# BerkIGuler/AdaFortiTran

Measured on AMD Instinct MI355X. Metric: OFDM frames/sec (120x14 grid, batch 128) + channel-estimation MSE vs reference, higher is better.
Workload: dtype f32; 1 GPU; C3: AdaFortiTran default config (6 layers, d=128, 4 heads, adaptive tokens), 120x14 grid, pilots 12x2; 128 frames per GPU per step; step = model(pilots_cpu, meta_cpu) through the module surface + device MSE partial; value = SURVEY 8(d)'s metric: H2D of pilots + meta INSIDE the step, output left on the device (= value_h2d_inclusive); the bare engine call on inputs resident in HBM is value_resident;; frames_per_gpu=128, global_batch=128, parallelism=frames sharded over 1 rank(s), lanes=1

## Files before the change

adafortitran_amd/csrc/attn16_device.h:

```cpp
#pragma once
#include <math.h>

#include <type_traits>

#include "attn_device.h"

namespace aft {

__device__ __forceinline__ f32x4 mfma16x4(float a, float b, f32x4 c) { return __builtin_amdgcn_mfma_f32_16x16x4f32(a, b, c, 0, 0, 0); }
__device__ __forceinline__ float srd_load1(Srd r, unsigned byte_off) {
    return __builtin_bit_cast(float, __builtin_amdgcn_raw_buffer_load_b32(r, byte_off, 0, 0));
}
__device__ __forceinline__ float groups_max(float x) {
    x = fmaxf(x, __shfl_xor(x, 16));
    return fmaxf(x, other_half(x));
}
__device__ __forceinline__ float groups_sum(float x) {
    x += __shfl_xor(x, 16);
    return x + other_half(x);
}

template <int TOK = 0, int HD = 16>
__device__ __forceinline__ void attn16_body(const float *__restrict__ q, const float *__restrict__ k, const float *__restrict__ vt,
                                            const float *__restrict__ qbias, float *__restrict__ out, int nblk, int tokens_rt,
                                            int tokpad_rt, int model_dim, float scale_log2e, const int first_task, const int total_waves,
                                            int ntasks, const int tail_task = -1) {
    int lane_l = threadIdx.x & 63;
    asm volatile("" : "+v"(lane_l));
    const int lane = lane_l, i = lane & 15, g = lane >> 4;
    const Srd qs = make_srd(q), ks = make_srd(k), vs = make_srd(vt), os = make_srd(out);
    const int tokens = TOK > 0 ? TOK : tokens_rt;
    const int tokpad = TOK > 0 ? (TOK + kTile - 1) / kTile * kTile : tokpad_rt;
    const int nkt = tokpad / kTile;
    const bool ragged = (tokens & (kTile - 1)) != 0;
    const unsigned blk_bytes = (unsigned)tokpad * kHeadDim * 4;
    static_assert(HD == 16 || HD == 8, "heads of 16 or 8 features");
    constexpr int NSUB = 32 / HD;
    auto first_block = [&](int task) { return (task / nkt) / NSUB; };
    auto sub_of = [&](int task) { return (task / nkt) & (NSUB - 1); };
    auto slot_of = [&](int sub) { return HD == 16 ? 2 * sub + (g >> 1) : sub; };
    const int vfeat = HD == 16 ? i : (i & 7);
    auto load_kq = [&](Srd src, int tile, f32x4 (&dst)[2], unsigned base, int sub) {
#pragma unroll
        for (int half = 0; half < 2; ++half)
            dst[half] = srd_load(src, base + (unsigned)(tile * 1024 + slot_of(sub) * 256 + (32 * (g & 1) + 16 * half + i) * 4) * 4u);
    };
    auto load_v = [&](int kt, f32x4 (&dst)[2], unsigned base, int sub) {
#pragma unroll
        for (int kb = 0; kb < 2; ++kb)
            dst[kb] = srd_load(vs, base + (unsigned)(kt * 1024 + (2 * kb + (g >> 1)) * 256 + (32 * (g & 1) + HD * sub + vfeat) * 4) * 4u);
    };
    auto mask_logits = [&](f32x4 (&sv)[2][2], int kt) {
#pragma unroll
        for (int kb = 0; kb < 2; ++kb)
#pragma unroll
            for (int v = 0; v < 4; ++v)
                if (kt * kTile + 16 * kb + 4 * g + v >= tokens) sv[kb][0][v] = sv[kb][1][v] = -INFINITY;
    };
    auto mask_values = [&](f32x4 (&vv)[2], int kt) {
#pragma unroll
        for (int kb = 0; kb < 2; ++kb)
#pragma unroll
            for (int v = 0; v < 4; ++v)
                if (kt * kTile + 16 * kb + 4 * g + v >= tokens) vv[kb][v] = 0.f;
    };
// ... 156 lines not shown
```

adafortitran_amd/csrc/attn_device.h:

```cpp
#pragma once
#include <math.h>

#include <type_traits>

#include "aft_internal.h"
#include "srd.h"

namespace aft {

#ifndef AFT_ATTN_WAVES
#define AFT_ATTN_WAVES 3
#endif

constexpr float kRescaleThreshold = 64.0f;
constexpr float kZeroRefThreshold = 32.0f;

__device__ __forceinline__ float other_half(float x) {
    const unsigned u = __builtin_bit_cast(unsigned, x);
    const auto r = __builtin_amdgcn_permlane32_swap(u, u, false, false);
    return __builtin_bit_cast(float, (threadIdx.x & 32) ? r[0] : r[1]);
}

__device__ __forceinline__ float max16(const f32x16 &v) {
    float m = __builtin_fmaxf(v[0], v[1]);
// ... 118 lines not shown
        }
#pragma unroll
        for (int e = 0; e < 16; ++e)
            if (kt * kTile + (e & 3) + 8 * (e >> 2) + 4 * h >= tokens) sv[e] = -INFINITY;
    };
    auto mask_values = [&](f32x4 (&vvb)[NB][4], int kt) {
      if (!BS && pad8) return;
#pragma unroll
      for (int b = 0; b < NB; ++b) {
        f32x4 (&vv)[4] = vvb[b];
        if constexpr (BS) {
#pragma unroll
            for (int sl = 0; sl < 4; ++sl) {
                bf16x8 e = __builtin_bit_cast(bf16x8, vv[sl]);
#pragma unroll
                for (int j = 0; j < 8; ++j)
                    if (kt * kTile + 16 * (sl >> 1) + 8 * (j >> 2) + 4 * h + (j & 3) >= tokens) e[j] = (__bf16)0.0f;
                vv[sl] = __builtin_bit_cast(f32x4, e);
            }
        } else {
#pragma unroll
            for (int g = 0; g < 4; ++g)
#pragma unroll
                for (int j = 0; j < 4; ++j)
                    if (kt * kTile + 8 * g + 4 * h + j >= tokens) vv[g][j] = 0.f;
        }
      }
    };

  const int rounds = SINK ? 1 : (ntasks + total_waves - 1) / total_waves + (tail_task >= 0 ? 1 : 0);
  int round = 0;
  int task = first_task < ntasks ? first_task : tail_task;
  f32x4 qreg[NQ][4], kcur[NQ][4], vcur[NB][4];
  if (task >= 0) {
      const unsigned hb0 = head_base(task);
      load_qk(qs, task % nkt, qreg, hb0, sub_of(task));
      load_qk(ks, 0, kcur, hb0, sub_of(task));
      load_tile(vs, 0, vcur, hb0, second_block_bytes(task));
  }
  for (; task >= 0; ++round) {
    ASTAMP(0);
#ifdef AFT_DIAG_STAMPS
    if (stamps && lane == 0) stamps[(size_t)task * 8 + 6] = __builtin_amdgcn_s_memrealtime();
#endif
    const int qt = task % nkt;
    const int pb = first_block(task);
    const int sub = sub_of(task);
    const unsigned hb = head_base(task);
    const unsigned vb1 = second_block_bytes(task);
    const int next_task = SINK || task >= ntasks ? -1 : (task + total_waves < ntasks ? task + total_waves : tail_task);
    const bool has_next = next_task >= 0;

    if constexpr (!BS) {
        const float *bq = qbias + (pb % nblk) * kHeadDim + 4 * h + (GEN ? 8 * sub : 0);
#pragma unroll
        for (int b = 0; b < NQ; ++b)
#pragma unroll
            for (int s = 0; s < 4; ++s)
                if (4 * b + s < (GEN ? NS : 4 * NB))
                    qreg[b][s] = (qreg[b][s] + *reinterpret_cast<const f32x4 *>(bq + 32 * b + 8 * s)) * scale_log2e;
    }
    if (ragged && qt == nkt - 1 && qt * kTile + r >= tokens) {
#pragma unroll
        for (int b = 0; b < NQ; ++b)
#pragma unroll
            for (int s = 0; s < 4; ++s)
                if (4 * b + s < (GEN ? NS : 4 * NB)) qreg[b][s] = f32x4{0.f, 0.f, 0.f, 0.f};
    }

    AttnRow<NB> st;
    f32x16 sA, sB;
    if constexpr (BS) sA = qk_tile_bs(kcur[0], qreg[0], true, 0.f, h);
    else sA = qk_tile<NQ, NMF>(kcur, qreg, true, a_one, 0.f);
    if (nkt > 1) load_qk(ks, 1, kcur, hb, sub);
    if (ragged && nkt == 1) { mask_logits(sA, 0); mask_values(vcur, 0); }
    {
        float m0 = max16(sA);
        m0 = fmaxf(m0, other_half(m0));
        if constexpr (BS) m0 = round_to_bf16(m0);
        st.zero_ref = !__any(fabsf(m0) > kZeroRefThreshold);
        st.m_ref = st.zero_ref ? 0.f : m0;
        if (!st.zero_ref) {
#pragma unroll
            for (int e = 0; e < 16; ++e) sA[e] -= m0;
        }
    }
#pragma unroll
    for (int b = 0; b < NB; ++b) st.oacc[b] = f32x16{0};
    st.lsum2 = f32x2{0.f, 0.f};
    ASTAMP(1);

    auto step = [&](auto fast, f32x16 &cur, f32x16 &nxt, int kt) {
        constexpr bool FAST = decltype(fast)::value;
        set_progress_priority((rounds - 1 - round) * nkt + (nkt - 1 - kt), rounds * nkt);
        const bool more = FAST || kt + 1 < nkt;
        if (more) {
            if constexpr (BS) nxt = qk_tile_bs(kcur[0], qreg[0], st.zero_ref, -st.m_ref, h);
            else nxt = qk_tile<NQ, NMF>(kcur, qreg, st.zero_ref, a_one, -st.m_ref);
            if (FAST || kt + 2 < nkt) load_qk(ks, kt + 2, kcur, hb, sub);
        } else if (has_next) {
            const unsigned hbn = head_base(next_task);
            load_qk(qs, next_task % nkt, qreg, hbn, sub_of(next_task));
            load_qk(ks, 0, kcur, hbn, sub_of(next_task));
        }
        const float tmax = max16(cur);
        if (__builtin_expect(__any(tmax > kRescaleThreshold), 0)) {
            const float tm = fmaxf(tmax, other_half(tmax));
            float grow = fmaxf(tm, 0.f);
            if constexpr (BS) grow = round_to_bf16(st.m_ref + grow) - st.m_ref;
            const float f = __builtin_amdgcn_exp2f(-grow);
            st.m_ref += grow;
            st.zero_ref = false;
#pragma unroll
// ... 94 lines not shown
```

adafortitran_amd/csrc/chain_device.h:

```cpp
#pragma once
#include "aft_internal.h"
#include "srd.h"

namespace aft {

template <int D>
struct ChainShape {
    static constexpr int WAVES = D / 32;
    static constexpr int THREADS = 64 * WAVES;
    static constexpr int XB = WAVES * 1024;
    static constexpr int HB = 2 * WAVES * 1024;
    static constexpr int ST = 32 * WAVES * 2;
    static constexpr int PAR = 4 * D;
    static constexpr size_t LDS_BYTES = sizeof(float) * (size_t)(XB + HB + ST + PAR);
};

struct ChainArgs {
    const float *attn;
    float *x;
    const float *wo, *w1, *w2, *wqkv;
    const float *bo, *b1, *b2, *g1, *be1, *g2, *be2;
    const float *bv;
    float *q, *k, *vt;
    int rows, tokens, tokpad, heads;
    int x_blocked;
    const float *lin2_w, *lin2_b;
    float *out6;
    int out6_features, out6_stride;
    const float *emb_conv, *emb_tok6, *emb_w1, *emb_b1, *emb_pos;
    int emb_S, emb_T, emb_p0, emb_p1, emb_K;
    unsigned long long *stamps;
    int tpp;
};

ChainArgs make_chain_args(const aft_config &c, const aft_layer_weights *mlp_w, const float *mlp_packed, const aft_layer_weights *qkv_w,
                          const float *qkv_packed, const float *attn, float *x, float *q, float *k, float *vt, int rows, int tokens,
                          int tokpad, const ChainFusion *fuse);

template <int NT, int PFS>
struct WRing {
    f32x4 b[PFS + 1][NT];
};


template <int NKB, int NT, int PFS, int TS>
__device__ __forceinline__ void ring_load(WRing<NT, PFS> &ring, Srd w, unsigned w_lane, int step) {
    const int kb = step >> 2, s = step & 3;
#pragma unroll
    for (int t = 0; t < NT; ++t)
        ring.b[step % (PFS + 1)][t] = srd_load_c(w, w_lane, (unsigned)((t * TS * NKB + kb) * 1024 + s * 256) * 4);
}

template <int NKB, int NT, int PFS, int TS>
__device__ __forceinline__ void gemm_preload(WRing<NT, PFS> &ring, Srd w, unsigned w_lane) {
#pragma unroll
    for (int p = 0; p < PFS && p < 4 * NKB; ++p) ring_load<NKB, NT, PFS, TS>(ring, w, w_lane, p);
    __builtin_amdgcn_sched_barrier(0);
}

template <int NKB, int NT, int PFS, int TS, unsigned NORMAL, class Act, unsigned ZERO = 0>
__device__ __forceinline__ void gemm_run(WRing<NT, PFS> &ring, Srd w, unsigned w_lane, f32x16 (&acc)[NT], Act act) {
#pragma unroll
    for (int step = 0; step < 4 * NKB; ++step) {
        if (step + PFS < 4 * NKB) ring_load<NKB, NT, PFS, TS>(ring, w, w_lane, step + PFS);
        __builtin_amdgcn_sched_barrier(0);
        const f32x4 a = act(step >> 2, step & 3);
#pragma unroll
        for (int t = 0; t < NT; ++t)
#pragma unroll
            for (int j = 0; j < 4; ++j) {
                const float wv = ring.b[step % (PFS + 1)][t][j];
                if (((ZERO >> t) & 1) && step == 0 && j == 0)
                    acc[t] = (NORMAL >> t) & 1 ? __builtin_amdgcn_mfma_f32_32x32x2f32(a[j], wv, f32x16{0}, 0, 0, 0)
                                               : __builtin_amdgcn_mfma_f32_32x32x2f32(wv, a[j], f32x16{0}, 0, 0, 0);
                else
                    acc[t] = (NORMAL >> t) & 1 ? __builtin_amdgcn_mfma_f32_32x32x2f32(a[j], wv, acc[t], 0, 0, 0)
                                               : __builtin_amdgcn_mfma_f32_32x32x2f32(wv, a[j], acc[t], 0, 0, 0);
            }
        __builtin_amdgcn_sched_barrier(0);
    }
}

__device__ __forceinline__ void bs_publish(float *buf, int block, int lane, const f32x16 &v) {
#pragma unroll
    for (int m = 0; m < 2; ++m) {
        const BsFrag f = bs_split(f32x4{v[8 * m], v[8 * m + 1], v[8 * m + 2], v[8 * m + 3]},
// ... 74 lines not shown

__device__ __forceinline__ f32x16 bias_acc(Srd bias, int f0, int h) {
    f32x16 acc;
#pragma unroll
    for (int s = 0; s < 4; ++s) {
        const f32x4 b = srd_load(bias, (unsigned)(f0 + 8 * s + 4 * h) * 4);
#pragma unroll
        for (int j = 0; j < 4; ++j) acc[4 * s + j] = b[j];
    }
    return acc;
}

#ifdef AFT_DIAG_STAMPS
#define STAMP(i)                                                                                               \
    do {                                                                                                       \
        if (a.stamps && tid == 0) a.stamps[(size_t)tile * 16 + (i)] = __builtin_amdgcn_s_memtime();    \
    } while (0)
#else
#define STAMP(i) do { } while (0)
#endif

struct ChainNoPre {
    __device__ __forceinline__ void operator()(int) const {}
};

template <int D, int ACT, bool MLP, bool QKV, bool BS = false, bool PT = false, class Pre = ChainNoPre>
__device__ __forceinline__ void chain_body(const ChainArgs &a, float *smem, const int tid_in, const int first_tile,
                                           const int tile_stride, const int tile_end, Pre pre = Pre{}) {
    using S = ChainShape<D>;
    constexpr int W = S::WAVES;
    static_assert(!PT || !BS, "plane-aligned tiles are instantiated for the fp32 body");
    int tid = tid_in;
    asm volatile("" : "+v"(tid));
    float *xb = smem;
    float *hb = xb + S::XB;
    float *stats = hb + S::HB;
    float *par = stats + S::ST;

    int lane = tid & 63;
    const int w = __builtin_amdgcn_readfirstlane(tid >> 6);
    int r = lane & 31, h = lane >> 5;
    const int fb = 32 * w;

    const Srd srd_wo = make_srd(a.wo), srd_w1 = make_srd(a.w1), srd_w2 = make_srd(a.w2), srd_wq = make_srd(a.wqkv);
    const Srd srd_attn = make_srd(a.attn), srd_x = make_srd(a.x);
    const Srd srd_bo = make_srd(a.bo), srd_b1 = make_srd(a.b1), srd_b2 = make_srd(a.b2);
    const Srd srd_q = make_srd(a.q), srd_k = make_srd(a.k), srd_vt = make_srd(a.vt);
    const unsigned wo_off = (unsigned)w * W * 1024 + lane * 4, w1_off = (unsigned)(2 * w) * W * 1024 + lane * 4;
    const unsigned w2_off = (unsigned)w * (2 * W) * 1024 + lane * 4;
    const unsigned wq_off = (unsigned)w * W * 1024 + lane * 4;
    const Srd srd_bv = make_srd(a.bv);

    if constexpr (MLP) {
        for (int i = tid; i < D; i += S::THREADS) {
            par[i] = a.g1[i];
            par[D + i] = a.be1[i];
            par[2 * D + i] = a.g2[i];
            par[3 * D + i] = a.be2[i];
        }
        __syncthreads();
    }
    constexpr int kEmbSteps = (kMaxPatchFeatures + 6 + 1) / 2;
    float *emb_w = hb + S::XB;
    int *emb_offs = reinterpret_cast<int *>(emb_w + D * (kMaxPatchFeatures + 6));
    if constexpr (!MLP) {
        if (a.emb_conv != nullptr) {
            const int pk = a.emb_p0 * a.emb_p1;
            for (int i = tid; i < D * a.emb_K; i += S::THREADS) emb_w[i] = a.emb_w1[i];
            for (int k = tid; k < a.emb_K; k += S::THREADS)
                emb_offs[k] = k < pk ? (k / a.emb_p1) * a.emb_T + k % a.emb_p1 : ~(k - pk);
            __syncthreads();
        }
    }
    const int ntiles = (a.rows + 31) / 32;
    const int rounds = (tile_end - first_tile + tile_stride - 1) / tile_stride;
    int round = 0;
#ifndef AFT_CHAIN_PFK
#define AFT_CHAIN_PFK 0
#endif
    constexpr int PFK = MLP ? (AFT_CHAIN_PFK < W ? AFT_CHAIN_PFK : W) : 0;
    constexpr bool AHEAD = AFT_CHAIN_PFK > 0;
    static_assert(!PT || !AHEAD, "plane-aligned tiles request a tile's operands at the tile's start");
    f32x4 of[MLP ? W : 1][4], xres[4];
    auto request_attn = [&](int t, int kb0, int kb1) {
        const unsigned ap = ((unsigned)t * W * 1024 + lane * 4) * 4;
#pragma unroll
        for (int kb = 0; kb < W; ++kb)
#pragma unroll
            for (int s = 0; s < 4; ++s)
                if (kb >= kb0 && kb < kb1) of[kb][s] = srd_load_c(srd_attn, ap, (unsigned)(kb * 1024 + s * 256) * 4);
    };
    auto request_x_pt = [&](int t, int valid) {
        const unsigned xr = ((unsigned)t * 32 * D + w * 1024 + (min(r, valid - 1) + 32 * h) * 4) * 4;
#pragma unroll
        for (int s = 0; s < 4; ++s) xres[s] = srd_load(srd_x, xr + 1024 * s);
    };
    auto request_x = [&](int t) {
        if (a.x_blocked) {
            const unsigned xr = ((unsigned)t * 32 * D + w * 1024 + lane * 4) * 4;
#pragma unroll
            for (int s = 0; s < 4; ++s) xres[s] = srd_load(srd_x, xr + 1024 * s);
        } else {
            const unsigned xr = ((unsigned)min(t * 32 + r, a.rows - 1) * D + fb + 4 * h) * 4;
#pragma unroll
            for (int s = 0; s < 4; ++s) xres[s] = srd_load(srd_x, xr + 32 * s);
        }
    };
    auto request_tile = [&](int t) {
        if constexpr (MLP) request_attn(t, 0, PFK);
        if (MLP || a.emb_conv == nullptr) request_x(t);
    };
    if (AHEAD && first_tile < ntiles) request_tile(first_tile);
    f32x16 emb_acc0;
    float emb_bv[kEmbSteps];
    auto emb_request = [&](int t) {
        int plane, tok;
        if constexpr (PT) {
            plane = t / a.tpp;
            tok = min((t - plane * a.tpp) * 32 + r, a.tokens - 1);
        } else {
            const int grow_n = min(t * 32 + r, a.rows - 1);
            plane = grow_n / a.tokens;
            tok = grow_n - plane * a.tokens;
        }
        const int tpr = a.emb_T / a.emb_p1, g = tok / tpr, tc = tok - g * tpr;
        const float *cplane = a.emb_conv + ((size_t)plane * a.emb_S + g * a.emb_p0) * a.emb_T + tc * a.emb_p1;
        const float *t6 = a.emb_tok6 ? a.emb_tok6 + ((size_t)(plane >> 1) * a.tokens + tok) * 6 : nullptr;
#pragma unroll
        for (int s = 0; s < 4; ++s) {
            const f32x4 b = *reinterpret_cast<const f32x4 *>(a.emb_b1 + fb + 8 * s + 4 * h);
            const f32x4 ps = *reinterpret_cast<const f32x4 *>(a.emb_pos + (size_t)tok * D + fb + 8 * s + 4 * h);
#pragma unroll
            for (int j = 0; j < 4; ++j) emb_acc0[4 * s + j] = b[j] + ps[j];
        }
#pragma unroll
        for (int st = 0; st < kEmbSteps; ++st) {
            const int k = 2 * st + h;
            emb_bv[st] = 0.f;
            if (k < a.emb_K) {
                const int off = emb_offs[k];
                emb_bv[st] = off >= 0 ? cplane[off] : t6[~off];
            }
        }
    };
    if constexpr (!MLP) {
        if (a.emb_conv != nullptr && first_tile < tile_end) emb_request(first_tile);
    }
    int pending_row0 = -1, pending_valid = 0;
    auto reduce_out6 = [&]() {
        const int P = a.out6_features;
        if (PT ? r < pending_valid : pending_row0 + r < a.rows) {
#pragma unroll
            for (int half = 0; half < 2; ++half) {
                const int f0 = 8 * half + 4 * h;
                if (f0 < P) {
                    f32x4 sum = *reinterpret_cast<const f32x4 *>(hb + lane * 8 + 4 * half);
#pragma unroll
                    for (int u = 1; u < W; ++u) {
                        const f32x4 t = *reinterpret_cast<const f32x4 *>(hb + (u * 64 + lane) * 8 + 4 * half);
                        sum += t;
                    }
#pragma unroll
                    for (int j = 0; j < 4; ++j) sum[j] += f0 + j < P ? a.lin2_b[f0 + j] : 0.f;
                    *reinterpret_cast<f32x4 *>(a.out6 + (size_t)(pending_row0 + r) * a.out6_stride + f0) = sum;
                }
            }
        }
    };
#pragma unroll 1
  for (int tile = first_tile; tile < tile_end; tile += tile_stride, ++round) {
    if constexpr (MLP && !QKV) {
        if (pending_row0 >= 0 && w == (round & (W - 1 < 3 ? W - 1 : 3))) reduce_out6();
    }
    pre(tile);
    if constexpr (PT && MLP) {
        int tid2 = tid_in;
        asm volatile("" : "+v"(tid2));
        lane = tid2 & 63;
        r = lane & 31;
        h = lane >> 5;
    }
#ifndef AFT_NO_PROGRESS_PRIORITY
    {
        const int left = rounds - 1 - round;
        if (left >= 3) __builtin_amdgcn_s_setprio(3);
        else if (left == 2) __builtin_amdgcn_s_setprio(2);
        else if (left == 1) __builtin_amdgcn_s_setprio(1);
        else __builtin_amdgcn_s_setprio(0);
    }
#endif
    const int row0 = tile * 32;
    const int grow = min(row0 + r, a.rows - 1);
    int plane_pt = 0, qt_pt = 0, valid_pt = 32;
    if constexpr (PT) {
        plane_pt = tile / a.tpp;
        qt_pt = tile - plane_pt * a.tpp;
        valid_pt = min(32, a.tokens - qt_pt * 32);
    }
    const bool row_ok = PT ? r < valid_pt : row0 + r < a.rows;
    const bool blocked = PT || a.x_blocked;
    const unsigned xrow = ((unsigned)grow * D + fb + 4 * h) * 4;
    unsigned lo = 0;
    asm volatile("" : "+v"(lo));
    const unsigned lo_lane = PT && MLP ? lo + lane * 4 : lo;
    const unsigned wo_lane = ((PT && MLP ? (unsigned)w * W * 1024 : wo_off) + lo_lane) * 4,
                   w1_lane = ((PT && MLP ? (unsigned)(2 * w) * W * 1024 : w1_off) + lo_lane) * 4,
                   w2_lane = ((PT && MLP ? (unsigned)w * (2 * W) * 1024 : w2_off) + lo_lane) * 4,
                   wq_lane = ((PT && MLP ? (unsigned)w * W * 1024 : wq_off) + lo_lane) * 4;
    STAMP(0);
#ifdef AFT_DIAG_STAMPS
    if (a.stamps && tid == 0) {
        a.stamps[(size_t)tile * 16 + 12] = __builtin_amdgcn_s_memrealtime();
        a.stamps[(size_t)tile * 16 + 14] = ((unsigned long long)__builtin_amdgcn_s_getreg((4 << 0) | (0 << 6) | (31 << 11)) << 32) |
                                           __builtin_amdgcn_s_getreg((20 << 0) | (0 << 6) | (31 << 11));
    }
#endif
#ifndef AFT_CHAIN_PFS
// ... 35 lines not shown
            bs_publish(xb, w, lane, cur);
        } else {
#pragma unroll
            for (int s = 0; s < 4; ++s)
                *reinterpret_cast<f32x4 *>(xb + (w * 4 + s) * 256 + lane * 4) = f32x4{cur[4 * s], cur[4 * s + 1], cur[4 * s + 2], cur[4 * s + 3]};
        }
        __syncthreads();
        STAMP(4);
        if constexpr (BS)
            gemm_run_bs<W, 2, PFF, 1, 0>(ring_ff, srd_w1, w1_lane, acc_h, [&](int kb, int m) { return bs_fetch(xb, kb, m, lane); });
        else
            gemm_run<W, 2, PFF, 1, 0>(ring_ff, srd_w1, w1_lane, acc_h, [&](int kb, int s) {
                return *reinterpret_cast<const f32x4 *>(xb + (kb * 4 + s) * 256 + lane * 4);
            });
        f32x16 acc_d[1] = {bias_acc(srd_b2, fb, h)};
        gemm_preload<2 * W, 1, PFD, 1>(ring_d, srd_w2, w2_lane);
        STAMP(5);
#pragma unroll
        for (int t = 0; t < 2; ++t) {
            f32x16 hid;
#pragma unroll
            for (int s = 0; s < 4; ++s) {
                const f32x2 g0 = activate2<ACT>(f32x2{acc_h[t][4 * s], acc_h[t][4 * s + 1]});
                const f32x2 g1 = activate2<ACT>(f32x2{acc_h[t][4 * s + 2], acc_h[t][4 * s + 3]});
                if constexpr (BS) {
                    hid[4 * s] = g0[0]; hid[4 * s + 1] = g0[1]; hid[4 * s + 2] = g1[0]; hid[4 * s + 3] = g1[1];
                } else {
                    *reinterpret_cast<f32x4 *>(hb + ((2 * w + t) * 4 + s) * 256 + lane * 4) = f32x4{g0[0], g0[1], g1[0], g1[1]};
                }
            }
            if constexpr (BS) bs_publish(hb, 2 * w + t, lane, hid);
        }
        __syncthreads();
        STAMP(6);
        if constexpr (BS)
            gemm_run_bs<2 * W, 1, PFD, 1, 0>(ring_d, srd_w2, w2_lane, acc_d, [&](int kb, int m) { return bs_fetch(hb, kb, m, lane); });
        else
            gemm_run<2 * W, 1, PFD, 1, 0>(ring_d, srd_w2, w2_lane, acc_d, [&](int kb, int s) {
                return *reinterpret_cast<const f32x4 *>(hb + (kb * 4 + s) * 256 + lane * 4);
            });
        if constexpr (QKV) gemm_preload<W, 3, PFQ, W>(ring_qkv, srd_wq, wq_lane);
#pragma unroll
        for (int e = 0; e < 16; ++e) cur[e] += acc_d[0][e];
        STAMP(7);
        layernorm_rows<D>(cur, stats, par + 2 * D + fb, par + 3 * D + fb, w, r, h);
        STAMP(8);
        if constexpr (!QKV) {
            if (AHEAD && tile + tile_stride < ntiles) request_tile(tile + tile_stride);
        }
        bool store_x = true;
        if constexpr (!QKV) {
            if (a.out6 != nullptr) {
                store_x = false;
                const int P = a.out6_features;
                f32x16 acc6 = f32x16{0};
#pragma unroll
                for (int s = 0; s < 4; ++s) {
                    f32x4 wv = {0.f, 0.f, 0.f, 0.f};
                    if (r < P) wv = *reinterpret_cast<const f32x4 *>(a.lin2_w + (size_t)r * D + fb + 8 * s + 4 * h);
#pragma unroll
                    for (int j = 0; j < 4; ++j) acc6 = __builtin_amdgcn_mfma_f32_32x32x2f32(wv[j], cur[4 * s + j], acc6, 0, 0, 0);
                }
                float *part = hb + (w * 64 + lane) * 8;
                *reinterpret_cast<f32x4 *>(part) = f32x4{acc6[0], acc6[1], acc6[2], acc6[3]};
                *reinterpret_cast<f32x4 *>(part + 4) = f32x4{acc6[4], acc6[5], acc6[6], acc6[7]};
                pending_row0 = PT ? plane_pt * a.tokens + qt_pt * 32 : row0;
                pending_valid = valid_pt;
            }
        }
        if (store_x && row_ok) {
            if (blocked) {
                const unsigned xblk = ((unsigned)row0 * D + w * 1024 + lane * 4) * 4;
#pragma unroll
                for (int s = 0; s < 4; ++s)
                    srd_store(srd_x, xblk + 1024 * s, f32x4{cur[4 * s], cur[4 * s + 1], cur[4 * s + 2], cur[4 * s + 3]});
            } else {
#pragma unroll
                for (int s = 0; s < 4; ++s)
                    srd_store(srd_x, xrow + 32 * s, f32x4{cur[4 * s], cur[4 * s + 1], cur[4 * s + 2], cur[4 * s + 3]});
            }
        }
    } else {
        gemm_preload<W, 3, PFQ, W>(ring_qkv, srd_wq, wq_lane);
        if (a.emb_conv == nullptr) {
            if (!AHEAD) request_x(tile);
#pragma unroll
            for (int s = 0; s < 4; ++s)
#pragma unroll
                for (int j = 0; j < 4; ++j) cur[4 * s + j] = xres[s][j];
        } else {
            f32x16 acc0 = emb_acc0;
            float av[kEmbSteps];
#pragma unroll
            for (int st = 0; st < kEmbSteps; ++st) {
                const int k = 2 * st + h;
                av[st] = k < a.emb_K ? emb_w[(fb + r) * a.emb_K + k] : 0.f;
            }
#pragma unroll
            for (int st = 0; st < kEmbSteps; ++st)
                if (2 * st < a.emb_K) acc0 = __builtin_amdgcn_mfma_f32_32x32x2f32(av[st], emb_bv[st], acc0, 0, 0, 0);
            cur = acc0;
            if (row_ok) {
                if (blocked) {
                    const unsigned xblk = ((unsigned)row0 * D + w * 1024 + lane * 4) * 4;
#pragma unroll
                    for (int s = 0; s < 4; ++s)
                        srd_store(srd_x, xblk + 1024 * s, f32x4{cur[4 * s], cur[4 * s + 1], cur[4 * s + 2], cur[4 * s + 3]});
                } else {
#pragma unroll
                    for (int s = 0; s < 4; ++s)
                        srd_store(srd_x, xrow + 32 * s, f32x4{cur[4 * s], cur[4 * s + 1], cur[4 * s + 2], cur[4 * s + 3]});
                }
            }
        }
    }

    if constexpr (QKV) {
        const float bias_v = __builtin_bit_cast(float, __builtin_amdgcn_raw_buffer_load_b32(srd_bv, (unsigned)(fb + r) * 4, 0, 0));
        float *xq = xb;
        if constexpr (!MLP) xq = (round & 1) ? hb : xb;
        if constexpr (BS) {
            bs_publish(xq, w, lane, cur);
        } else {
#pragma unroll
            for (int s = 0; s < 4; ++s)
                *reinterpret_cast<f32x4 *>(xq + (w * 4 + s) * 256 + lane * 4) = f32x4{cur[4 * s], cur[4 * s + 1], cur[4 * s + 2], cur[4 * s + 3]};
        }
        __syncthreads();
        STAMP(9);
        f32x16 vinit;
#pragma unroll
        for (int e = 0; e < 16; ++e) vinit[e] = bias_v;
        f32x16 acc[3];
        acc[2] = vinit;
        if constexpr (BS) {
            acc[0] = bias_acc(make_srd(a.bv - 2 * D), fb, h);
            auto xq_bs = [&](int kb, int m) { return bs_fetch(xq, kb, m, lane); };
            gemm_run_bs<W, 3, PFQ, W, 0x4, decltype(xq_bs), 0x2>(ring_qkv, srd_wq, wq_lane, acc, xq_bs);
        } else {
            auto xq_frag = [&](int kb, int s) { return *reinterpret_cast<const f32x4 *>(xq + (kb * 4 + s) * 256 + lane * 4); };
            gemm_run<W, 3, PFQ, W, 0x4, decltype(xq_frag), 0x3>(ring_qkv, srd_wq, wq_lane, acc, xq_frag);
        }
        STAMP(10);
        if (AHEAD && tile + tile_stride < ntiles) request_tile(tile + tile_stride);
        if constexpr (!MLP) {
            if (a.emb_conv != nullptr && tile + tile_stride < tile_end) emb_request(tile + tile_stride);
        }
        if constexpr (PT) {
            const unsigned ph_base = (unsigned)(plane_pt * a.heads + w) * ((unsigned)a.tokpad * kHeadDim) + (unsigned)qt_pt * 1024;
            if (row_ok) {
#pragma unroll
                for (int s = 0; s < 4; ++s) {
                    srd_store(srd_q, (ph_base + lane * 4 + s * 256) * 4, f32x4{acc[0][4 * s], acc[0][4 * s + 1], acc[0][4 * s + 2], acc[0][4 * s + 3]});
// ... 156 lines not shown
```

adafortitran_amd/csrc/k_chain.hip:

```cpp
#include <algorithm>
#include <cstdio>
#include <cstdlib>
#include <vector>

#include "chain_device.h"
#include "pack_device.h"

#ifndef AFT_CHAIN_MANY_MAX_D
#define AFT_CHAIN_MANY_MAX_D 96
#endif

namespace aft {

template <int D, int ACT, bool MLP, bool QKV>
__global__ __launch_bounds__(D * 2, D <= 128 ? 3 : 2) void chain_kernel(const ChainArgs a) {
    extern __shared__ __attribute__((aligned(16))) float smem[];
    chain_body<D, ACT, MLP, QKV>(a, smem, threadIdx.x, blockIdx.x, gridDim.x, (a.rows + 31) / 32);
}


template <int D, int ACT, bool MLP, bool QKV>
__global__ __launch_bounds__(D * 2, D <= 128 ? 3 : 2) void chain_split_kernel(const ChainArgs a) {
    extern __shared__ __attribute__((aligned(16))) float smem[];
    chain_body<D, ACT, MLP, QKV, true>(a, smem, threadIdx.x, blockIdx.x, gridDim.x, (a.rows + 31) / 32);
// ... 105 lines not shown
                       smin, ssum / (r1 - r0), smax, emin, esum / (r1 - r0), emax);
            }
        }
        return hipGetLastError();
    }
#endif
    hipLaunchKernelGGL((chain_kernel<D, ACT, MLP, QKV>), dim3(blocks), dim3(S::THREADS), lds, st, args);
    return hipGetLastError();
}

size_t packed_layer_floats(int d) { return (size_t)8 * d * d; }

__global__ __launch_bounds__(256) void pack_weights_kernel(const WeightsDev w, float *__restrict__ packed, int d,
                                                           int num_layers, int split) {
    pack_weights_vec(w, packed, d, 0, num_layers, split, (size_t)blockIdx.x * 256 + threadIdx.x);
}

hipError_t launch_pack_weights(const aft_config &c, const aft_layer_weights *layers, float *packed, int count, hipStream_t st) {
    for (int first = 0; first < count; first += kLayerWindow) {
        const int n = std::min(kLayerWindow, count - first);
        WeightsDev win{};
        for (int i = 0; i < n; ++i) win.layers[i] = layers[first + i];
        const size_t vecs = packed_layer_floats(c.model_dim) * n / 4;
        hipLaunchKernelGGL(pack_weights_kernel, dim3((unsigned)((vecs + 255) / 256)), dim3(256), 0, st, win,
                           packed + packed_layer_floats(c.model_dim) * first, c.model_dim, n, c.precision == AFT_PRECISION_BF16X3 ? 1 : 0);
        hipError_t e = hipGetLastError();
        if (e != hipSuccess) return e;
    }
    return hipSuccess;
}

template <int D, int ACT>
static hipError_t launch_chain_t(const ChainArgs &args, bool mlp, bool qkv, hipStream_t st) {
    if (mlp && qkv) return launch_chain_v<D, ACT, true, true>(args, st);
    if (mlp) return launch_chain_v<D, ACT, true, false>(args, st);
    return launch_chain_v<D, ACT, false, true>(args, st);
}

ChainArgs make_chain_args(const aft_config &c, const aft_layer_weights *m, const float *m_packed, const aft_layer_weights *qw,
                          const float *q_packed, const float *attn, float *x, float *q, float *k, float *vt, int rows, int tokens,
                          int tokpad, const ChainFusion *fuse) {
    const size_t dd = (size_t)c.model_dim * c.model_dim;
    ChainArgs a{};
    if (fuse != nullptr && fuse->out6 != nullptr && m != nullptr && qw == nullptr) {
        a.lin2_w = fuse->lin2_w; a.lin2_b = fuse->lin2_b; a.out6 = fuse->out6;
        a.out6_features = c.patch_scs * c.patch_symbols;
        a.out6_stride = out6_stride(c);
    }
    if (fuse != nullptr && fuse->conv_enhanced != nullptr && m == nullptr) {
        a.emb_conv = fuse->conv_enhanced; a.emb_tok6 = fuse->tokens6; a.emb_w1 = fuse->lin1_w; a.emb_b1 = fuse->lin1_b;
        a.emb_pos = fuse->pos;
        a.emb_S = c.num_scs; a.emb_T = c.num_symbols; a.emb_p0 = c.patch_scs; a.emb_p1 = c.patch_symbols;
        a.emb_K = c.patch_scs * c.patch_symbols + (fuse->tokens6 ? 6 : 0);
    }
    a.attn = attn;
    a.x = x;
    a.x_blocked = fuse != nullptr && fuse->x_blocked ? 1 : 0;
    if (m != nullptr) {
        a.wo = m_packed + 3 * dd; a.bo = m->out_proj_b;
        a.w1 = m_packed + 4 * dd; a.b1 = m->lin1_b;
        a.w2 = m_packed + 6 * dd; a.b2 = m->lin2_b;
        a.g1 = m->norm1_w; a.be1 = m->norm1_b;
        a.g2 = m->norm2_w; a.be2 = m->norm2_b;
    }
    if (qw != nullptr) {
        a.wqkv = q_packed;
        a.bv = qw->in_proj_b + 2 * c.model_dim;
    }
    a.q = q; a.k = k; a.vt = vt;
    a.rows = rows; a.tokens = tokens; a.tokpad = tokpad;
    a.heads = c.model_dim / kHeadDim;
    return a;
}

hipError_t launch_chain(const aft_config &c, const aft_layer_weights *m, const float *m_packed,
                        const aft_layer_weights *qw, const float *q_packed,
                        const float *attn, float *x, float *q, float *k, float *vt, int rows, int tokens,
                        int tokpad, hipStream_t st, const ChainFusion *fuse) {
    const ChainArgs a = make_chain_args(c, m, m_packed, qw, q_packed, attn, x, q, k, vt, rows, tokens, tokpad, fuse);
    const bool gelu = c.activation == AFT_ACT_GELU;
    const bool mlp = m != nullptr, qkv = qw != nullptr;
    if (c.precision == AFT_PRECISION_BF16X3) {
        if (c.model_dim == 128)
            return gelu ? launch_chain_split_t<128, AFT_ACT_GELU>(a, mlp, qkv, st) : launch_chain_split_t<128, AFT_ACT_RELU>(a, mlp, qkv, st);
        if (c.model_dim == 256)
            return gelu ? launch_chain_split_t<256, AFT_ACT_GELU>(a, mlp, qkv, st) : launch_chain_split_t<256, AFT_ACT_RELU>(a, mlp, qkv, st);
        return hipErrorInvalidValue;
    }
#define AFT_CHAIN_DIM(DD) \
    if (c.model_dim == DD) return gelu ? launch_chain_t<DD, AFT_ACT_GELU>(a, mlp, qkv, st) : launch_chain_t<DD, AFT_ACT_RELU>(a, mlp, qkv, st);
    AFT_CHAIN_DIM(32) AFT_CHAIN_DIM(96) AFT_CHAIN_DIM(160) AFT_CHAIN_DIM(224)
#undef AFT_CHAIN_DIM
    if (c.model_dim == 64)
        return gelu ? launch_chain_t<64, AFT_ACT_GELU>(a, mlp, qkv, st) : launch_chain_t<64, AFT_ACT_RELU>(a, mlp, qkv, st);
    if (c.model_dim == 192)
        return gelu ? launch_chain_t<192, AFT_ACT_GELU>(a, mlp, qkv, st) : launch_chain_t<192, AFT_ACT_RELU>(a, mlp, qkv, st);
    if (c.model_dim == 128)
        return gelu ? launch_chain_t<128, AFT_ACT_GELU>(a, mlp, qkv, st) : launch_chain_t<128, AFT_ACT_RELU>(a, mlp, qkv, st);
    if (c.model_dim == 256)
        return gelu ? launch_chain_t<256, AFT_ACT_GELU>(a, mlp, qkv, st) : launch_chain_t<256, AFT_ACT_RELU>(a, mlp, qkv, st);
    return hipErrorInvalidValue;
}

}
```

adafortitran_amd/csrc/k_layer.hip:

```cpp
#include <algorithm>

#include "attn_device.h"
#include "chain_device.h"

namespace aft {

struct LayerArgs {
    ChainArgs c;
    const float *aq, *ak, *avt, *qbias;
    float scale_log2e;
    int planes;
};

template <int D, int TOK>
struct LayerAttention {
    const LayerArgs &a;
    float *sink;
    __device__ __forceinline__ void operator()(int tile) const {
        const int w = __builtin_amdgcn_readfirstlane(threadIdx.x >> 6);
        const int plane = tile / a.c.tpp, qt = tile - plane * a.c.tpp;
        const int task = (plane * (D / kHeadDim) + w) * a.c.tpp + qt;
        attn_body<false, kHeadDim, TOK, true>(a.aq, a.ak, a.avt, a.qbias, nullptr, D / kHeadDim, a.c.tokens, a.c.tokpad, D, a.scale_log2e, task,
                                              1 << 30, task + 1, nullptr, -1, sink + w * 1024);
        __syncthreads();
    }
};

template <int D, int ACT, bool QKV, int TOK>
__global__ __launch_bounds__(D * 2, 3) void layer_kernel(const LayerArgs a) {
    extern __shared__ __attribute__((aligned(16))) float smem[];
    using S = ChainShape<D>;
    int vblock = blockIdx.x;
    if ((gridDim.x & 7) == 0) vblock = (blockIdx.x & 7) * (gridDim.x >> 3) + (blockIdx.x >> 3);
    chain_body<D, ACT, true, QKV, false, true>(a.c, smem, threadIdx.x, vblock, gridDim.x, a.planes * a.c.tpp,
                                               LayerAttention<D, TOK>{a, smem + S::XB + S::XB});
}

template <int D>
__global__ __launch_bounds__(D * 2, 3) void chain_plane_tiles_kernel(const ChainArgs a, int planes) {
    extern __shared__ __attribute__((aligned(16))) float smem[];
    int vblock = blockIdx.x;
    if ((gridDim.x & 7) == 0) vblock = (blockIdx.x & 7) * (gridDim.x >> 3) + (blockIdx.x >> 3);
    chain_body<D, AFT_ACT_RELU, false, true, false, true>(a, smem, threadIdx.x, vblock, gridDim.x, planes * a.tpp);
}

template <class K, class A, class... Rest>
static hipError_t launch_plane_tiles(K kernel, const A &args, int planes, int tpp, hipStream_t st, PerDeviceOnce &lds_attr, Rest... rest) {
    using S = ChainShape<128>;
    hipError_t ea = ensure_dynamic_lds(lds_attr, reinterpret_cast<const void *>(kernel), S::LDS_BYTES);
    if (ea != hipSuccess) return ea;
    const int blocks = std::min(planes * tpp, current_device_cus() * 3);
    hipLaunchKernelGGL(kernel, dim3(blocks), dim3(S::THREADS), S::LDS_BYTES, st, args, rest...);
    return hipGetLastError();
}

bool layer_fused_ok(const aft_config &c) {
    return packed_engine_ok(c) && c.precision == AFT_PRECISION_F32 && c.model_dim == 128 && c.num_head * kHeadDim == c.model_dim &&
           tokens_of(c) >= kTile;
}

hipError_t launch_chain_plane_tiles(const aft_config &c, const aft_layer_weights *qw, const float *q_packed, float *x, float *q, float *k,
                                    float *vt, int planes, int tokens, int tokpad, hipStream_t st, const ChainFusion *fuse) {
    if (!layer_fused_ok(c) || fuse == nullptr || fuse->conv_enhanced == nullptr) return hipErrorInvalidValue;
    ChainArgs a = make_chain_args(c, nullptr, nullptr, qw, q_packed, nullptr, x, q, k, vt, planes * tokens, tokens, tokpad, fuse);
    a.tpp = tokpad / kTile;
    static PerDeviceOnce once;
    return launch_plane_tiles(chain_plane_tiles_kernel<128>, a, planes, a.tpp, st, once, planes);
}

template <int ACT, bool QKV, int TOK>
static hipError_t launch_layer_v(const LayerArgs &a, hipStream_t st) {
    static PerDeviceOnce once;
    return launch_plane_tiles(layer_kernel<128, ACT, QKV, TOK>, a, a.planes, a.c.tpp, st, once);
}
template <int ACT, bool QKV>
static hipError_t launch_layer_t(const LayerArgs &a, hipStream_t st) {
    return a.c.tokens == 280 ? launch_layer_v<ACT, QKV, 280>(a, st) : launch_layer_v<ACT, QKV, 0>(a, st);
}

hipError_t launch_layer(const aft_config &c, const aft_layer_weights *m, const float *m_packed, const aft_layer_weights *qw,
                        const float *q_packed, float *x, float *q, const float *k_in, const float *vt_in, float *k_out, float *vt_out,
                        int planes, int tokens, int tokpad, hipStream_t st, const ChainFusion *fuse) {
    if (!layer_fused_ok(c) || m == nullptr || k_in == k_out || vt_in == vt_out) return hipErrorInvalidValue;
    LayerArgs a{};
    a.c = make_chain_args(c, m, m_packed, qw, q_packed, nullptr, x, q, k_out, vt_out, planes * tokens, tokens, tokpad, fuse);
    a.c.tpp = tokpad / kTile;
    a.aq = q; a.ak = k_in; a.avt = vt_in;
    a.qbias = m->in_proj_b;
    a.scale_log2e = 1.4426950408889634f / sqrtf((float)kHeadDim);
    a.planes = planes;
    const bool gelu = c.activation == AFT_ACT_GELU;
    if (qw != nullptr) return gelu ? launch_layer_t<AFT_ACT_GELU, true>(a, st) : launch_layer_t<AFT_ACT_RELU, true>(a, st);
    return gelu ? launch_layer_t<AFT_ACT_GELU, false>(a, st) : launch_layer_t<AFT_ACT_RELU, false>(a, st);
}

}
```

adafortitran_amd/csrc/srd.h:

```cpp
#pragma once
#include "aft_internal.h"

namespace aft {

using Srd = __amdgpu_buffer_rsrc_t;
__device__ __forceinline__ Srd make_srd(const float *p) {
    return __builtin_amdgcn_make_buffer_rsrc(const_cast<float *>(p), 0, 0x7fffffff, 0x00020000);
}
__device__ __forceinline__ f32x4 srd_load(Srd r, unsigned byte_off) {
    return __builtin_bit_cast(f32x4, __builtin_amdgcn_raw_buffer_load_b128(r, byte_off, 0, 0));
}
__device__ __forceinline__ f32x4 srd_load_c(Srd r, unsigned byte_off, unsigned const_off) {
    return __builtin_bit_cast(f32x4, __builtin_amdgcn_raw_buffer_load_b128(r, byte_off + (const_off & 0xfffu), const_off & ~0xfffu, 0));
}
__device__ __forceinline__ void srd_store(Srd r, unsigned byte_off, f32x4 v) {
    __builtin_amdgcn_raw_buffer_store_b128(__builtin_bit_cast(decltype(__builtin_amdgcn_raw_buffer_load_b128(r, 0, 0, 0)), v), r, byte_off, 0, 0);
}

using bf16x8 = __attribute__((__vector_size__(8 * sizeof(__bf16)))) __bf16;
struct BsFrag {
    f32x4 hi, lo;
};
__device__ __forceinline__ BsFrag bs_split(f32x4 x0, f32x4 x1) {
    bf16x8 hi, lo;
#pragma unroll
    for (int j = 0; j < 8; ++j) {
        const float x = j < 4 ? x0[j] : x1[j - 4];
        hi[j] = (__bf16)x;
        lo[j] = (__bf16)(x - (float)hi[j]);
    }
    return BsFrag{__builtin_bit_cast(f32x4, hi), __builtin_bit_cast(f32x4, lo)};
}

}
```

Before: 84230 frames/s.

## Use bounded buffer loads and incremental indexing in fused embedding prologue

Switches the embedding gather, LayerNorm params, lin2 head and sink-attention q-bias loads from flat pointer loads to buffer-resource loads with explicit sizes. Out-of-range accesses then return zero, which removes the conv-vs-tok6 branch: both sources are loaded and OR-combined. Plane/token indices are advanced incrementally, and division uses a precomputed 24-bit multiply. Kernel arguments are re-read from the kernarg segment to ease scalar register pressure. This adds host-side exactness checks that reject unsupported shapes, and relies on the LayerArgs layout starting with ChainArgs.

```diff
diff --git a/adafortitran_amd/csrc/attn16_device.h b/adafortitran_amd/csrc/attn16_device.h
--- a/adafortitran_amd/csrc/attn16_device.h
+++ b/adafortitran_amd/csrc/attn16_device.h
@@ -8,9 +8,6 @@
 namespace aft {
 
 __device__ __forceinline__ f32x4 mfma16x4(float a, float b, f32x4 c) { return __builtin_amdgcn_mfma_f32_16x16x4f32(a, b, c, 0, 0, 0); }
-__device__ __forceinline__ float srd_load1(Srd r, unsigned byte_off) {
-    return __builtin_bit_cast(float, __builtin_amdgcn_raw_buffer_load_b32(r, byte_off, 0, 0));
-}
 __device__ __forceinline__ float groups_max(float x) {
     x = fmaxf(x, __shfl_xor(x, 16));
     return fmaxf(x, other_half(x));
diff --git a/adafortitran_amd/csrc/attn_device.h b/adafortitran_amd/csrc/attn_device.h
--- a/adafortitran_amd/csrc/attn_device.h
+++ b/adafortitran_amd/csrc/attn_device.h
@@ -194,6 +194,12 @@
     const bool has_next = next_task >= 0;
 
     if constexpr (!BS) {
+        if constexpr (SINK) {
+            const Srd bqs = make_srd(qbias, (unsigned)model_dim * 4);
+            const unsigned bq = (unsigned)((pb % nblk) * kHeadDim + 4 * h) * 4;
+#pragma unroll
+            for (int s = 0; s < 4; ++s) qreg[0][s] = (qreg[0][s] + srd_load(bqs, bq + 32 * s)) * scale_log2e;
+        } else {
         const float *bq = qbias + (pb % nblk) * kHeadDim + 4 * h + (GEN ? 8 * sub : 0);
 #pragma unroll
         for (int b = 0; b < NQ; ++b)
@@ -201,6 +207,7 @@
             for (int s = 0; s < 4; ++s)
                 if (4 * b + s < (GEN ? NS : 4 * NB))
                     qreg[b][s] = (qreg[b][s] + *reinterpret_cast<const f32x4 *>(bq + 32 * b + 8 * s)) * scale_log2e;
+        }
     }
     if (ragged && qt == nkt - 1 && qt * kTile + r >= tokens) {
 #pragma unroll
diff --git a/adafortitran_amd/csrc/chain_device.h b/adafortitran_amd/csrc/chain_device.h
--- a/adafortitran_amd/csrc/chain_device.h
+++ b/adafortitran_amd/csrc/chain_device.h
@@ -29,9 +29,23 @@
     int out6_features, out6_stride;
     const float *emb_conv, *emb_tok6, *emb_w1, *emb_b1, *emb_pos;
     int emb_S, emb_T, emb_p0, emb_p1, emb_K;
+    unsigned emb_conv_bytes, emb_tok6_bytes, emb_div_mul;
+    int emb_tpr;
     unsigned long long *stamps;
     int tpp;
 };
+
+using KernArgPtr = const char __attribute__((address_space(4))) *;
+__device__ __forceinline__ KernArgPtr chain_args_here() {
+    KernArgPtr kp = (KernArgPtr)__builtin_amdgcn_kernarg_segment_ptr();
+    asm volatile("" : "+s"(kp));
+    return kp;
+}
+#define AFT_CHAIN_ARG(kp, field) \
+    (*reinterpret_cast<const decltype(ChainArgs::field) __attribute__((address_space(4))) *>((kp) + offsetof(ChainArgs, field)))
+
+constexpr int kEmbDivShift = 23;
+constexpr unsigned kSrdNowhere = 0x80000000u;
 
 ChainArgs make_chain_args(const aft_config &c, const aft_layer_weights *mlp_w, const float *mlp_packed, const aft_layer_weights *qkv_w,
                           const float *qkv_packed, const float *attn, float *x, float *q, float *k, float *vt, int rows, int tokens,
@@ -212,23 +226,26 @@
     const Srd srd_bv = make_srd(a.bv);
 
     if constexpr (MLP) {
+        const Srd srd_g1 = make_srd(a.g1, D * 4), srd_be1 = make_srd(a.be1, D * 4), srd_g2 = make_srd(a.g2, D * 4), srd_be2 = make_srd(a.be2, D * 4);
         for (int i = tid; i < D; i += S::THREADS) {
-            par[i] = a.g1[i];
-            par[D + i] = a.be1[i];
-            par[2 * D + i] = a.g2[i];
-            par[3 * D + i] = a.be2[i];
+            par[i] = srd_load1(srd_g1, (unsigned)i * 4);
+            par[D + i] = srd_load1(srd_be1, (unsigned)i * 4);
+            par[2 * D + i] = srd_load1(srd_g2, (unsigned)i * 4);
+            par[3 * D + i] = srd_load1(srd_be2, (unsigned)i * 4);
         }
         __syncthreads();
     }
     constexpr int kEmbSteps = (kMaxPatchFeatures + 6 + 1) / 2;
     float *emb_w = hb + S::XB;
-    int *emb_offs = reinterpret_cast<int *>(emb_w + D * (kMaxPatchFeatures + 6));
+    uint2 *emb_offs = reinterpret_cast<uint2 *>(emb_w + D * (kMaxPatchFeatures + 6));
     if constexpr (!MLP) {
         if (a.emb_conv != nullptr) {
             const int pk = a.emb_p0 * a.emb_p1;
-            for (int i = tid; i < D * a.emb_K; i += S::THREADS) emb_w[i] = a.emb_w1[i];
-            for (int k = tid; k < a.emb_K; k += S::THREADS)
-                emb_offs[k] = k < pk ? (k / a.emb_p1) * a.emb_T + k % a.emb_p1 : ~(k - pk);
+            const Srd srd_w1e = make_srd(a.emb_w1, (unsigned)(D * a.emb_K) * 4);
+            for (int i = tid; i < D * a.emb_K; i += S::THREADS) emb_w[i] = srd_load1(srd_w1e, (unsigned)i * 4);
+            for (int k = tid; k < 2 * kEmbSteps; k += S::THREADS)
+                emb_offs[k] = make_uint2(k < pk ? (unsigned)((k / a.emb_p1) * a.emb_T + k % a.emb_p1) * 4 : kSrdNowhere,
+                                         k >= pk && k < a.emb_K ? (unsigned)(k - pk) * 4 : kSrdNowhere);
             __syncthreads();
         }
     }
@@ -272,34 +289,57 @@
     };
     if (AHEAD && first_tile < ntiles) request_tile(first_tile);
     f32x16 emb_acc0;
-    float emb_bv[kEmbSteps];
+    float emb_bv[kEmbSteps], emb_bt[kEmbSteps];
+    const int emb_period = PT ? a.tpp : a.tokens, emb_unit = PT ? tile_stride : 32 * tile_stride;
+    int emb_plane = 0, emb_at = 0, emb_dplane = 0, emb_dat = 0;
+    if constexpr (!MLP) {
+        if (a.emb_conv != nullptr) {
+            const int at0 = PT ? first_tile : 32 * first_tile;
+            emb_plane = at0 / emb_period;
+            emb_at = at0 - emb_plane * emb_period;
+            emb_dplane = emb_unit / emb_period;
+            emb_dat = emb_unit - emb_dplane * emb_period;
+        }
+    }
     auto emb_request = [&](int t) {
-        int plane, tok;
+        int plane = emb_plane, tok;
         if constexpr (PT) {
-            plane = t / a.tpp;
-            tok = min((t - plane * a.tpp) * 32 + r, a.tokens - 1);
-        } else {
-            const int grow_n = min(t * 32 + r, a.rows - 1);
-            plane = grow_n / a.tokens;
-            tok = grow_n - plane * a.tokens;
-        }
-        const int tpr = a.emb_T / a.emb_p1, g = tok / tpr, tc = tok - g * tpr;
-        const float *cplane = a.emb_conv + ((size_t)plane * a.emb_S + g * a.emb_p0) * a.emb_T + tc * a.emb_p1;
-        const float *t6 = a.emb_tok6 ? a.emb_tok6 + ((size_t)(plane >> 1) * a.tokens + tok) * 6 : nullptr;
+            tok = min(emb_at * 32 + r, a.tokens - 1);
+        } else {
+            tok = emb_at + min(t * 32 + r, a.rows - 1) - t * 32;
+            if (tok >= a.tokens) { tok -= a.tokens; ++plane; }
+            if (a.tokens < kTile)
+                while (tok >= a.tokens) { tok -= a.tokens; ++plane; }
+        }
+        emb_plane += emb_dplane;
+        emb_at += emb_dat;
+        if (emb_at >= emb_period) { emb_at -= emb_period; ++emb_plane; }
+        const KernArgPtr kp = chain_args_here();
+        const int eS = AFT_CHAIN_ARG(kp, emb_S), eT = AFT_CHAIN_ARG(kp, emb_T), ep0 = AFT_CHAIN_ARG(kp, emb_p0), ep1 = AFT_CHAIN_ARG(kp, emb_p1);
+        const int emb_k = AFT_CHAIN_ARG(kp, emb_K), etpr = AFT_CHAIN_ARG(kp, emb_tpr);
+        const unsigned g = __umul24((unsigned)tok, AFT_CHAIN_ARG(kp, emb_div_mul)) >> kEmbDivShift, tc = (unsigned)tok - __umul24(g, (unsigned)etpr);
+        const unsigned crow = ((unsigned)plane * (unsigned)(eS * eT) + __umul24(g, (unsigned)(ep0 * eT)) + __umul24(tc, (unsigned)ep1)) * 4;
+        const unsigned trow = ((unsigned)(plane >> 1) * (unsigned)a.tokens + (unsigned)tok) * 24;
+        const unsigned prow = ((unsigned)tok * D + fb + 4 * h) * 4;
+        const Srd srd_conv = make_srd(AFT_CHAIN_ARG(kp, emb_conv), AFT_CHAIN_ARG(kp, emb_conv_bytes));
+        const Srd srd_t6 = make_srd(AFT_CHAIN_ARG(kp, emb_tok6), AFT_CHAIN_ARG(kp, emb_tok6_bytes));
+        const Srd srd_pos = make_srd(AFT_CHAIN_ARG(kp, emb_pos), (unsigned)a.tokens * D * 4), srd_b1e = make_srd(AFT_CHAIN_ARG(kp, emb_b1), D * 4);
 #pragma unroll
         for (int s = 0; s < 4; ++s) {
-            const f32x4 b = *reinterpret_cast<const f32x4 *>(a.emb_b1 + fb + 8 * s + 4 * h);
-            const f32x4 ps = *reinterpret_cast<const f32x4 *>(a.emb_pos + (size_t)tok * D + fb + 8 * s + 4 * h);
+            const f32x4 b = srd_load(srd_b1e, (unsigned)(fb + 8 * s + 4 * h) * 4);
+            const f32x4 ps = srd_load(srd_pos, prow + 32 * s);
 #pragma unroll
             for (int j = 0; j < 4; ++j) emb_acc0[4 * s + j] = b[j] + ps[j];
         }
 #pragma unroll
+        for (int e = 0; e < 16; ++e) asm volatile("" : "+v"(emb_acc0[e]));
+#pragma unroll
         for (int st = 0; st < kEmbSteps; ++st) {
-            const int k = 2 * st + h;
-            emb_bv[st] = 0.f;
-            if (k < a.emb_K) {
-                const int off = emb_offs[k];
-                emb_bv[st] = off >= 0 ? cplane[off] : t6[~off];
+            emb_bv[st] = emb_bt[st] = 0.f;
+            if (2 * st < emb_k) {
+                const uint2 off = emb_offs[2 * st + h];
+                emb_bv[st] = srd_load1(srd_conv, crow + off.x);
+                emb_bt[st] = srd_load1(srd_t6, trow + off.y);
             }
         }
     };
@@ -308,7 +348,10 @@
     }
     int pending_row0 = -1, pending_valid = 0;
     auto reduce_out6 = [&]() {
-        const int P = a.out6_features;
+        const KernArgPtr kp = chain_args_here();
+        const int P = AFT_CHAIN_ARG(kp, out6_features), stride6 = AFT_CHAIN_ARG(kp, out6_stride);
+        const Srd srd_l2b = make_srd(AFT_CHAIN_ARG(kp, lin2_b), (unsigned)P * 4);
+        const Srd srd_out6 = make_srd(AFT_CHAIN_ARG(kp, out6), (unsigned)a.rows * (unsigned)stride6 * 4);
         if (PT ? r < pending_valid : pending_row0 + r < a.rows) {
 #pragma unroll
             for (int half = 0; half < 2; ++half) {
@@ -321,8 +364,8 @@
                         sum += t;
                     }
 #pragma unroll
-                    for (int j = 0; j < 4; ++j) sum[j] += f0 + j < P ? a.lin2_b[f0 + j] : 0.f;
-                    *reinterpret_cast<f32x4 *>(a.out6 + (size_t)(pending_row0 + r) * a.out6_stride + f0) = sum;
+                    for (int j = 0; j < 4; ++j) sum[j] += srd_load1(srd_l2b, (unsigned)(f0 + j) * 4);
+                    srd_store(srd_out6, ((unsigned)(pending_row0 + r) * (unsigned)stride6 + f0) * 4, sum);
                 }
             }
         }
@@ -464,12 +507,14 @@
         if constexpr (!QKV) {
             if (a.out6 != nullptr) {
                 store_x = false;
-                const int P = a.out6_features;
+                const KernArgPtr kp = chain_args_here();
+                const int P = AFT_CHAIN_ARG(kp, out6_features);
                 f32x16 acc6 = f32x16{0};
+                const Srd srd_l2w = make_srd(AFT_CHAIN_ARG(kp, lin2_w), (unsigned)(P * D) * 4);
+                const unsigned l2row = r < P ? (unsigned)(r * D + fb + 4 * h) * 4 : kSrdNowhere;
 #pragma unroll
                 for (int s = 0; s < 4; ++s) {
-                    f32x4 wv = {0.f, 0.f, 0.f, 0.f};
-                    if (r < P) wv = *reinterpret_cast<const f32x4 *>(a.lin2_w + (size_t)r * D + fb + 8 * s + 4 * h);
+                    const f32x4 wv = srd_load(srd_l2w, l2row + 32 * s);
 #pragma unroll
                     for (int j = 0; j < 4; ++j) acc6 = __builtin_amdgcn_mfma_f32_32x32x2f32(wv[j], cur[4 * s + j], acc6, 0, 0, 0);
                 }
@@ -503,14 +548,18 @@
         } else {
             f32x16 acc0 = emb_acc0;
             float av[kEmbSteps];
+            const int emb_k = AFT_CHAIN_ARG(chain_args_here(), emb_K);
 #pragma unroll
             for (int st = 0; st < kEmbSteps; ++st) {
                 const int k = 2 * st + h;
-                av[st] = k < a.emb_K ? emb_w[(fb + r) * a.emb_K + k] : 0.f;
+                av[st] = k < emb_k ? emb_w[(fb + r) * emb_k + k] : 0.f;
             }
 #pragma unroll
             for (int st = 0; st < kEmbSteps; ++st)
-                if (2 * st < a.emb_K) acc0 = __builtin_amdgcn_mfma_f32_32x32x2f32(av[st], emb_bv[st], acc0, 0, 0, 0);
+                if (2 * st < emb_k) {
+                    const float bv = __builtin_bit_cast(float, __builtin_bit_cast(unsigned, emb_bv[st]) | __builtin_bit_cast(unsigned, emb_bt[st]));
+                    acc0 = __builtin_amdgcn_mfma_f32_32x32x2f32(av[st], bv, acc0, 0, 0, 0);
+                }
             cur = acc0;
             if (row_ok) {
                 if (blocked) {
diff --git a/adafortitran_amd/csrc/k_chain.hip b/adafortitran_amd/csrc/k_chain.hip
--- a/adafortitran_amd/csrc/k_chain.hip
+++ b/adafortitran_amd/csrc/k_chain.hip
@@ -181,6 +181,14 @@
         a.emb_pos = fuse->pos;
         a.emb_S = c.num_scs; a.emb_T = c.num_symbols; a.emb_p0 = c.patch_scs; a.emb_p1 = c.patch_symbols;
         a.emb_K = c.patch_scs * c.patch_symbols + (fuse->tokens6 ? 6 : 0);
+        const size_t planes = (size_t)rows / tokens;
+        a.emb_conv_bytes = (unsigned)(planes * c.num_scs * c.num_symbols * sizeof(float));
+        a.emb_tok6_bytes = fuse->tokens6 ? (unsigned)(planes / 2 * tokens * 6 * sizeof(float)) : 0u;
+        a.emb_tpr = c.num_symbols / c.patch_symbols;
+        const unsigned long long mul = (1ull << kEmbDivShift) / a.emb_tpr + 1;
+        const bool exact = (unsigned long long)tokens * a.emb_tpr <= (1ull << kEmbDivShift) &&
+                           (unsigned long long)(tokens - 1) * mul < (1ull << 32) && mul < (1ull << 24);
+        a.emb_div_mul = exact ? (unsigned)mul : 0u;
     }
     a.attn = attn;
     a.x = x;
@@ -207,6 +215,7 @@
                         const float *attn, float *x, float *q, float *k, float *vt, int rows, int tokens,
                         int tokpad, hipStream_t st, const ChainFusion *fuse) {
     const ChainArgs a = make_chain_args(c, m, m_packed, qw, q_packed, attn, x, q, k, vt, rows, tokens, tokpad, fuse);
+    if (a.emb_conv != nullptr && a.emb_div_mul == 0) return hipErrorInvalidValue;
     const bool gelu = c.activation == AFT_ACT_GELU;
     const bool mlp = m != nullptr, qkv = qw != nullptr;
     if (c.precision == AFT_PRECISION_BF16X3) {
diff --git a/adafortitran_amd/csrc/k_layer.hip b/adafortitran_amd/csrc/k_layer.hip
--- a/adafortitran_amd/csrc/k_layer.hip
+++ b/adafortitran_amd/csrc/k_layer.hip
@@ -11,6 +11,7 @@
     float scale_log2e;
     int planes;
 };
+static_assert(offsetof(LayerArgs, c) == 0, "chain_body re-reads its ChainArgs from the start of the kernel-argument segment (AFT_CHAIN_ARG)");
 
 template <int D, int TOK>
 struct LayerAttention {
@@ -64,6 +65,7 @@
     if (!layer_fused_ok(c) || fuse == nullptr || fuse->conv_enhanced == nullptr) return hipErrorInvalidValue;
     ChainArgs a = make_chain_args(c, nullptr, nullptr, qw, q_packed, nullptr, x, q, k, vt, planes * tokens, tokens, tokpad, fuse);
     a.tpp = tokpad / kTile;
+    if (a.emb_div_mul == 0) return hipErrorInvalidValue;
     static PerDeviceOnce once;
     return launch_plane_tiles(chain_plane_tiles_kernel<128>, a, planes, a.tpp, st, once, planes);
 }
diff --git a/adafortitran_amd/csrc/srd.h b/adafortitran_amd/csrc/srd.h
--- a/adafortitran_amd/csrc/srd.h
+++ b/adafortitran_amd/csrc/srd.h
@@ -6,6 +6,12 @@
 using Srd = __amdgpu_buffer_rsrc_t;
 __device__ __forceinline__ Srd make_srd(const float *p) {
     return __builtin_amdgcn_make_buffer_rsrc(const_cast<float *>(p), 0, 0x7fffffff, 0x00020000);
+}
+__device__ __forceinline__ Srd make_srd(const float *p, unsigned bytes) {
+    return __builtin_amdgcn_make_buffer_rsrc(const_cast<float *>(p), 0, (int)bytes, 0x00020000);
+}
+__device__ __forceinline__ float srd_load1(Srd r, unsigned byte_off) {
+    return __builtin_bit_cast(float, __builtin_amdgcn_raw_buffer_load_b32(r, byte_off, 0, 0));
 }
 __device__ __forceinline__ f32x4 srd_load(Srd r, unsigned byte_off) {
     return __builtin_bit_cast(f32x4, __builtin_amdgcn_raw_buffer_load_b128(r, byte_off, 0, 0));
```

Result: no change. 84340 frames/s (median of 3 runs) (+0.1%).
